# ak110/object_detector

Measured on AMD Instinct MI355X. Metric: images_per_sec, higher is better.
Workload: dtype f16

## Files before the change

### object_detector_amd/csrc/conv_bneck.hip

```cpp
#include <stdlib.h>

#include "conv_common.h"

namespace {

struct BneckKP {
  const f16* x;
  const f16* w1;
  const float* s1;
  const float* b1;
  const f16* w3;
  const float* s3;
  const float* b3;
  f16* out;
  const f16* zero;
  int B, H, W;
  int k1stride, k3stride;
  int act;
  float alpha;
  int tiles_x, tiles_y;
};

template <int CPR>
static __device__ __forceinline__ int bn_swz(int row) {
  return CPR == 16 ? ((row & 7) << 1) : (CPR == 8 ? (row & 7) : 3 * ((row >> 2) & 1));
}

template <int ACT>
static __device__ __forceinline__ float bn_act(float v, float alpha) {
  if (ACT == OD_ACT_LEAKY) return od_leaky(v, alpha);
  if (ACT == OD_ACT_ELU) return v > 0.f ? v : alpha * od_expm1_fast(v);
  return v;
}

static __device__ __forceinline__ __amdgpu_buffer_rsrc_t bn_make_rsrc(const void* base, unsigned bytes) {
  return __builtin_amdgcn_make_buffer_rsrc((void*)base, 0, (int)bytes, 0x00020000);
}
static __device__ __forceinline__ void bn_buffer_dma(__amdgpu_buffer_rsrc_t rs, int voff, int soff, char* lds) {
  __builtin_amdgcn_raw_ptr_buffer_load_lds(rs, (__attribute__((address_space(3))) void*)lds, 16, voff, soff, 0, 0);
}

template <int C>
struct BneckCfg {
  static constexpr int CM = C / 2;
  static constexpr int RBX = 2 * C, RBT = C;
  static constexpr int CPX = RBX / 16, CPT = RBT / 16;
  static constexpr int WW = 18, NWP = WW * WW, NWF = 21;
  static constexpr int XW_BYTES = NWF * 16 * RBX;
  static constexpr int TW_BYTES = NWP * RBT;
  static constexpr int W1_BYTES = CM * RBX;
  static constexpr int W3TAP = C * RBT;
  static constexpr bool RESIDENT = (C == 64);
  static constexpr int NXW = RESIDENT ? 2 : 1;
  static constexpr int OFF_XW = 0, OFF_TW = NXW * XW_BYTES, OFF_W1 = OFF_TW + TW_BYTES;
  static constexpr int OFF_W3 = OFF_W1 + W1_BYTES;
  static constexpr int LDS_BYTES = RESIDENT ? OFF_W3 + 9 * W3TAP : OFF_W3 + W3TAP;
  static constexpr int NSLOT = 7;
  static_assert(RESIDENT || (W3TAP == W1_BYTES && 5 * W3TAP <= XW_BYTES), "ring slots must fit the freed regions");
  static constexpr int NF1 = CM / 16, KS1 = C / 32;
  static constexpr int NF3 = C / 16, KS3 = CM / 32;
  static constexpr int NFW = NF3 / 2;
  static constexpr int TAP_DMAS = C * CPT / 512;
  static __host__ __device__ constexpr int slot_off(int slot) {
    return slot == 0 ? OFF_W3 : (slot == 1 ? OFF_W1 : OFF_XW + (slot - 2) * W3TAP);
  }
};

template <int C, int ACT = OD_ACT_LEAKY>
__global__ __launch_bounds__(C == 64 ? 768 : 512, C == 64 ? 3 : 2) void od_bneck(BneckKP p, int ntiles) {
  using Cf = BneckCfg<C>;
  constexpr bool LOADERS = (C == 64);
  constexpr int CM = Cf::CM, RBX = Cf::RBX, RBT = Cf::RBT, CPX = Cf::CPX, CPT = Cf::CPT, WW = Cf::WW, NWP = Cf::NWP;
  constexpr int NF1 = Cf::NF1, KS1 = Cf::KS1, KS3 = Cf::KS3, NFW = Cf::NFW;
  extern __shared__ __attribute__((aligned(16))) char smem[];

  const int tid = threadIdx.x;
  const int lane = tid & 63;
  const int wave = __builtin_amdgcn_readfirstlane(tid >> 6);
  const int l15 = lane & 15, lq = lane >> 4;
  const int tpi = p.tiles_x * p.tiles_y;

  constexpr int XWT = LOADERS ? 256 : 512;
  constexpr int XWR = (NWP * CPX + XWT - 1) / XWT;
  const int xtid = LOADERS ? tid - 512 : tid, xwave = LOADERS ? wave - 8 : wave;
  int xw_rel[XWR], xw_wyx[XWR];
#pragma unroll
  for (int r = 0; r < XWR; ++r) {
    const int q = r * XWT + xtid;
    const int wp = q / CPX, pc = q - wp * CPX;
    const int wy = wp / WW, wx = wp - wy * WW;
    xw_rel[r] = ((wy - 1) * p.W + (wx - 1)) * C + (pc ^ bn_swz<CPX>(wp)) * 8;
    xw_wyx[r] = (q >= 0 && q < NWP * CPX && xtid >= 0) ? ((wy << 8) | wx) : -1;
  }
  auto issue_xwin = [&](int tile, int buf) {
    const int b = tile / tpi;
    const int trem = tile - b * tpi;
    const int tyi = trem / p.tiles_x, txi = trem - tyi * p.tiles_x;
    const int y0 = tyi * 16, x0 = txi * 16;
    const f16* org = p.x + ((long long)(b * p.H + y0) * p.W + x0) * C;
#pragma unroll
    for (int r = 0; r < XWR; ++r) {
      if (xw_wyx[r] >= 0) {
        const int y = y0 - 1 + (xw_wyx[r] >> 8), x = x0 - 1 + (xw_wyx[r] & 255);
        const bool ok = (unsigned)y < (unsigned)p.H && (unsigned)x < (unsigned)p.W;
        const f16* src = ok ? org + xw_rel[r] : p.zero;
        glds16(src, smem + Cf::OFF_XW + buf * Cf::XW_BYTES + (r * XWT + xwave * 64) * 16);
      }
    }
  };
  constexpr int TAPR = (C * CPT + 511) / 512;
  int tap_voff[TAPR];
#pragma unroll
  for (int r = 0; r < TAPR; ++r) {
    const int q = r * 512 + tid;
    const int n = q / CPT, pc = q - n * CPT;
    tap_voff[r] = q < C * CPT ? (n * p.k3stride + (pc ^ bn_swz<CPT>(n)) * 8) * 2 : (int)0x80000000;
  }
  const __amdgpu_buffer_rsrc_t rs_w3 = bn_make_rsrc(p.w3, 256u * (unsigned)p.k3stride * 2u);
  auto load_tap = [&](int tap, int dst_off) {
#pragma unroll
    for (int r = 0; r < TAPR; ++r) {
      char* dst = smem + dst_off + (r * 512 + wave * 64) * 16;
      if ((r + 1) * 512 <= C * CPT) {
        bn_buffer_dma(rs_w3, tap_voff[r], tap * CM * 2, dst);
      } else if (r * 512 + wave * 64 < C * CPT) {
        bn_buffer_dma(rs_w3, tap_voff[r], tap * CM * 2, dst);
      }
    }
  };

  int tile = blockIdx.x;
  if (tile >= ntiles) return;
  if (LOADERS && wave >= 8) {
    issue_xwin(tile, 0);
    wait_vmcnt<0>();
    __syncthreads();
    int curl = 0;
#pragma unroll 1
    for (; tile < ntiles; tile += (int)gridDim.x) {
      if (tile + (int)gridDim.x < ntiles) issue_xwin(tile + (int)gridDim.x, curl ^ 1);
      __builtin_amdgcn_s_barrier();
      wait_vmcnt<0>();
      __builtin_amdgcn_s_barrier();
      curl ^= 1;
    }
    return;
  }
  if (!LOADERS) issue_xwin(tile, 0);
#pragma unroll 1
  for (int q = tid; q < CM * CPX + 63; q += 512) {
    if (q < CM * CPX) {
      const int n = q / CPX, pc = q - n * CPX;
      const int lc = pc ^ bn_swz<CPX>(n);
      glds16(p.w1 + (long long)n * p.k1stride + lc * 8, smem + Cf::OFF_W1 + (q - lane) * 16);
    }
  }
  if (Cf::RESIDENT) {
#pragma unroll 1
    for (int tap = 0; tap < 9; ++tap) load_tap(tap, Cf::OFF_W3 + tap * Cf::W3TAP);
  } else {
    load_tap(0, Cf::slot_off(0));
  }
  wait_vmcnt<0>();
  __syncthreads();

  const int wm = wave >> 1, wn = wave & 1;
  int boff[NFW][KS3];
#pragma unroll
  for (int j = 0; j < NFW; ++j)
#pragma unroll
    for (int ks = 0; ks < KS3; ++ks) {
      const int row = (wn * NFW + j) * 16 + l15;
      boff[j][ks] = row * RBT + (((ks * 4 + lq) ^ bn_swz<CPT>(row)) * 16);
    }

  int cur = 0;
#pragma unroll 1
  for (; tile < ntiles; tile += (int)gridDim.x) {
    const int b = tile / tpi;
    const int trem = tile - b * tpi;
    const int tyi = trem / p.tiles_x, txi = trem - tyi * p.tiles_x;
    const int y0 = tyi * 16, x0 = txi * 16;
    const char* xw = smem + Cf::OFF_XW + cur * Cf::XW_BYTES;

    {
    f16x8 wb1[NF1][KS1];
  #pragma unroll
    for (int j = 0; j < NF1; ++j)
  #pragma unroll
      for (int ks = 0; ks < KS1; ++ks) {
        const int row = j * 16 + l15;
        wb1[j][ks] = *(const f16x8*)(smem + Cf::OFF_W1 + row * RBX + (((ks * 4 + lq) ^ bn_swz<CPX>(row)) * 16));
      }
    float sc1[NF1][4], bi1[NF1][4];
  #pragma unroll
    for (int j = 0; j < NF1; ++j) {
      const f32x4 s = *(const f32x4*)(p.s1 + j * 16 + lq * 4), bb = *(const f32x4*)(p.b1 + j * 16 + lq * 4);
  #pragma unroll
      for (int e = 0; e < 4; ++e) {
        sc1[j][e] = s[e];
        bi1[j][e] = bb[e];
      }
    }
  #pragma unroll 1
      for (int f = wave; f < Cf::NWF; f += 8) {
        const int wp = f * 16 + l15;
        f32x4 acc1[NF1];
  #pragma unroll
        for (int j = 0; j < NF1; ++j) acc1[j] = f32x4{0.f, 0.f, 0.f, 0.f};
  #pragma unroll
        for (int ks = 0; ks < KS1; ++ks) {
          const f16x8 xa = *(const f16x8*)(xw + wp * RBX + (((ks * 4 + lq) ^ bn_swz<CPX>(wp)) * 16));
  #pragma unroll
          for (int j = 0; j < NF1; ++j) acc1[j] = __builtin_amdgcn_mfma_f32_16x16x32_f16(wb1[j][ks], xa, acc1[j], 0, 0, 0);
        }
        if (wp < NWP) {
          const int wy = wp / WW, wx = wp - wy * WW;
          const bool inside = (unsigned)(y0 - 1 + wy) < (unsigned)p.H && (unsigned)(x0 - 1 + wx) < (unsigned)p.W;
  #pragma unroll
          for (int j = 0; j < NF1; ++j) {
            f16x4 h;
  #pragma unroll
            for (int e = 0; e < 4; ++e) {
              const float v = bn_act<ACT>(acc1[j][e] * sc1[j][e] + bi1[j][e], p.alpha);
              h[e] = inside ? (f16)v : (f16)0.f;
            }
            const int lc = j * 2 + (lq >> 1);
            *(f16x4*)(smem + Cf::OFF_TW + wp * RBT + ((lc ^ bn_swz<CPT>(wp)) * 16) + (lq & 1) * 8) = h;
          }
        }
      }

    }

    f16x8 resv[NFW / 2][4];
    if (!Cf::RESIDENT) {
#pragma unroll
      for (int pr = 0; pr < NFW / 2; ++pr) {
        const int ch = (wn * NFW + 2 * pr + (lq & 1)) * 16 + (lq >> 1) * 8;
#pragma unroll
        for (int i = 0; i < 4; ++i) {
          const int wrow = (wm * 4 + i + 1) * WW + 1 + l15;
          resv[pr][i] = *(const f16x8*)(xw + wrow * RBX + (((ch >> 3) ^ bn_swz<CPX>(wrow)) * 16));
        }
      }
    }
    __syncthreads();

    if (Cf::RESIDENT) {
      if (!LOADERS && tile + (int)gridDim.x < ntiles) issue_xwin(tile + (int)gridDim.x, cur ^ 1);
    } else {
#pragma unroll
      for (int k = 1; k <= 6; ++k) load_tap((k % 3) * 3 + k / 3, Cf::slot_off(k));
    }

    f32x4 acc[4][NFW];
#pragma unroll
    for (int i = 0; i < 4; ++i)
#pragma unroll
      for (int j = 0; j < NFW; ++j) acc[i][j] = f32x4{0.f, 0.f, 0.f, 0.f};

    f16x8 xa[6][KS3];
    auto load_col = [&](int dx) {
#pragma unroll
      for (int k = 0; k < 6; ++k) {
        const int wrow = (wm * 4 + k) * WW + dx + l15;
#pragma unroll
        for (int ks = 0; ks < KS3; ++ks)
          xa[k][ks] = *(const f16x8*)(smem + Cf::OFF_TW + wrow * RBT + (((ks * 4 + lq) ^ bn_swz<CPT>(wrow)) * 16));
      }
    };
    auto do_tap = [&](int dy, int wbase) {
#pragma unroll
      for (int ks = 0; ks < KS3; ++ks) {
        f16x8 wb[NFW];
#pragma unroll
        for (int j = 0; j < NFW; ++j) wb[j] = *(const f16x8*)(smem + wbase + boff[j][ks]);
#pragma unroll
        for (int i = 0; i < 4; ++i)
#pragma unroll
          for (int j = 0; j < NFW; ++j)
            acc[i][j] = __builtin_amdgcn_mfma_f32_16x16x32_f16(wb[j], xa[i + dy][ks], acc[i][j], 0, 0, 0);
      }
    };
    if (Cf::RESIDENT) {
#pragma unroll
      for (int dx = 0; dx < 3; ++dx) {
        load_col(dx);
#pragma unroll
        for (int dy = 0; dy < 3; ++dy) do_tap(dy, Cf::OFF_W3 + (dy * 3 + dx) * Cf::W3TAP);
      }
    } else {
      constexpr int D = Cf::TAP_DMAS;
      load_col(0);
      do_tap(0, Cf::slot_off(0));
      wait_vmcnt<5 * D>();
      __builtin_amdgcn_s_barrier();
      load_tap(1 * 3 + 2, Cf::slot_off(0));
      do_tap(1, Cf::slot_off(1));
      wait_vmcnt<5 * D>();
      __builtin_amdgcn_s_barrier();
      load_tap(2 * 3 + 2, Cf::slot_off(1));
      do_tap(2, Cf::slot_off(2));
      wait_vmcnt<5 * D>();
      __builtin_amdgcn_s_barrier();
      load_col(1);
      do_tap(0, Cf::slot_off(3));
      wait_vmcnt<4 * D>();
      __builtin_amdgcn_s_barrier();
      do_tap(1, Cf::slot_off(4));
      wait_vmcnt<3 * D>();
      __builtin_amdgcn_s_barrier();
      do_tap(2, Cf::slot_off(5));
      wait_vmcnt<2 * D>();
      __builtin_amdgcn_s_barrier();
      load_col(2);
      do_tap(0, Cf::slot_off(6));
      wait_vmcnt<1 * D>();
      __builtin_amdgcn_s_barrier();
      do_tap(1, Cf::slot_off(0));
      wait_vmcnt<0>();
      __builtin_amdgcn_s_barrier();
      do_tap(2, Cf::slot_off(1));
    }

    od_mfma_results_ready();
#pragma unroll
    for (int pr = 0; pr < NFW / 2; ++pr) {
      const int ch = (wn * NFW + 2 * pr + (lq & 1)) * 16 + (lq >> 1) * 8;
      float sc[8], bi[8];
      {
        const f32x4 s0 = *(const f32x4*)(p.s3 + ch), s1 = *(const f32x4*)(p.s3 + ch + 4);
        const f32x4 b0 = *(const f32x4*)(p.b3 + ch), b1 = *(const f32x4*)(p.b3 + ch + 4);
#pragma unroll
        for (int e = 0; e < 4; ++e) {
          sc[e] = s0[e];
          sc[4 + e] = s1[e];
          bi[e] = b0[e];
          bi[4 + e] = b1[e];
        }
      }
#pragma unroll
      for (int i = 0; i < 4; ++i) {
        const int ty = wm * 4 + i;
        f16x8 r;
        if (Cf::RESIDENT) {
          const int wrow = (ty + 1) * WW + 1 + l15;
          r = *(const f16x8*)(xw + wrow * RBX + (((ch >> 3) ^ bn_swz<CPX>(wrow)) * 16));
        } else {
          r = resv[pr][i];
        }
        float v[8];
#pragma unroll
        for (int e = 0; e < 4; ++e) {
          float a = acc[i][2 * pr][e], bq = acc[i][2 * pr + 1][e];
          od_permlane16_swap(a, bq);
          v[e] = a;
          v[4 + e] = bq;
        }
        f16x8 h;
#pragma unroll
        for (int e = 0; e < 8; ++e) h[e] = (f16)(bn_act<ACT>(v[e] * sc[e] + bi[e], p.alpha) + (float)r[e]);
        *(f16x8*)(p.out + ((long long)(b * p.H + y0 + ty) * p.W + x0 + l15) * C + ch) = h;
      }
    }
    if (Cf::RESIDENT) {
      if (!LOADERS) wait_vmcnt<(NFW / 2) * 4>();
      __syncthreads();
      cur ^= 1;
    }
  }
}

}

extern "C" int od_bottleneck_supported(int H, int W, int C) {
  return (C == 64 || C == 128) && H > 0 && W > 0 && (H % 16) == 0 && (W % 16) == 0;
}

int od_bottleneck_prepare(od_ctx* ctx, const od_bneck_desc* d, od_launches* L) {
  OD_REQUIRE(ctx && d, "od_bottleneck_fwd: null ctx/desc");
  OD_REQUIRE(d->x && d->w1 && d->scale1 && d->bias1 && d->w3 && d->scale3 && d->bias3 && d->out,
             "od_bottleneck_fwd: null tensor");
  OD_REQUIRE(od_bottleneck_supported(d->H, d->W, d->C),
             "od_bottleneck_fwd: needs C in {64, 128} and H, W multiples of 16 (got C=%d, %dx%d)", d->C, d->H, d->W);
  OD_REQUIRE(d->B > 0 && (long long)d->B * d->H * d->W * d->C < (1LL << 31), "od_bottleneck_fwd: bad batch / tensor too large");
  OD_REQUIRE(d->act >= OD_ACT_LINEAR && d->act <= OD_ACT_ELU, "od_bottleneck_fwd: bad act");
  OD_REQUIRE(d->act != OD_ACT_LEAKY || (d->alpha >= 0.f && d->alpha <= 1.f), "od_bottleneck_fwd: leaky slope must be in [0, 1]");
  BneckKP p;
  p.x = (const f16*)d->x;
  p.w1 = (const f16*)d->w1;
  p.s1 = d->scale1;
  p.b1 = d->bias1;
  p.w3 = (const f16*)d->w3;
  p.s3 = d->scale3;
  p.b3 = d->bias3;
  p.out = (f16*)d->out;
  p.zero = (const f16*)ctx->zero_page;
  p.B = d->B;
  p.H = d->H;
  p.W = d->W;
  p.k1stride = od_round_up(d->C, 64);
  p.k3stride = od_round_up(9 * (d->C / 2), 64);
  p.act = d->act;
  p.alpha = d->alpha;
  p.tiles_x = d->W / 16;
  p.tiles_y = d->H / 16;
  static_assert(OD_ACT_LINEAR == 0 && OD_ACT_LEAKY == 1 && OD_ACT_ELU == 2, "kernel table order");
#define OD_BN(C, ACT) {(const void*)&od_bneck<C, ACT>, "od_bneck<" #C ", " #ACT ">"}
  static const struct {
    const void* fn;
    const char* name;
  } kernels[2][3] = {{OD_BN(64, 0), OD_BN(64, 1), OD_BN(64, 2)}, {OD_BN(128, 0), OD_BN(128, 1), OD_BN(128, 2)}};
#undef OD_BN
  const auto& k = kernels[d->C == 128][d->act];
  const int lds = d->C == 64 ? BneckCfg<64>::LDS_BYTES : BneckCfg<128>::LDS_BYTES;
  if (int rc = od_ensure_lds(ctx, k.fn, (size_t)lds)) return rc;
  const int ntiles = d->B * p.tiles_x * p.tiles_y;
  const int cus = ctx->num_cu;
  const int grid = d->C == 64 ? (ntiles < cus ? ntiles : cus) : ntiles;
  return od_add_launch(L, {k.name, od_issue_kp_int<BneckKP>, k.fn, dim3((unsigned)grid), dim3(d->C == 64 ? 768 : 512), (size_t)lds},
                       od_kp_int<BneckKP>{p, ntiles});
}

extern "C" int od_bottleneck_fwd(od_ctx* ctx, const od_bneck_desc* d, void* stream) {
  return od_prepare_issue(stream, od_bottleneck_prepare, ctx, d);
}
```

Baseline: 21060.

## Make C=128 bottleneck persistent with next-tile window prefetch into freed ring slots

For the C=128 bottleneck kernel, the grid becomes persistent (capped at CU count). Each CTA now streams the next tile's input window into ring slots freed during the 3x3 tap loop, then reloads tap 0 and the 1x1 weights at the end of the iteration. Scale and bias vectors are cached in LDS instead of being read from global memory every tile. The aim is to hide the input-window and weight load latency behind MFMA work, at the cost of much more intricate vmcnt bookkeeping and tighter LDS usage.

```diff
diff --git a/object_detector_amd/csrc/conv_bneck.hip b/object_detector_amd/csrc/conv_bneck.hip
--- a/object_detector_amd/csrc/conv_bneck.hip
+++ b/object_detector_amd/csrc/conv_bneck.hip
@@ -54,9 +54,13 @@
   static constexpr int NXW = RESIDENT ? 2 : 1;
   static constexpr int OFF_XW = 0, OFF_TW = NXW * XW_BYTES, OFF_W1 = OFF_TW + TW_BYTES;
   static constexpr int OFF_W3 = OFF_W1 + W1_BYTES;
-  static constexpr int LDS_BYTES = RESIDENT ? OFF_W3 + 9 * W3TAP : OFF_W3 + W3TAP;
+  static constexpr int OFF_SB = OFF_W3 + W3TAP;
+  static constexpr int LDS_BYTES = RESIDENT ? OFF_W3 + 9 * W3TAP : OFF_SB + (2 * CM + 2 * C) * 4;
   static constexpr int NSLOT = 7;
   static_assert(RESIDENT || (W3TAP == W1_BYTES && 5 * W3TAP <= XW_BYTES), "ring slots must fit the freed regions");
+  static constexpr int XROUNDS = (NWP * CPX + 511) / 512;
+  static_assert(RESIDENT || (CPX == 16 && W3TAP == 2 * 8192 && (XROUNDS - 1) * 8192 == 5 * W3TAP && LDS_BYTES <= 160 * 1024),
+                "window rounds must map onto ring slots 2-6");
   static constexpr int NF1 = CM / 16, KS1 = C / 32;
   static constexpr int NF3 = C / 16, KS3 = CM / 32;
   static constexpr int NFW = NF3 / 2;
@@ -65,6 +69,22 @@
     return slot == 0 ? OFF_W3 : (slot == 1 ? OFF_W1 : OFF_XW + (slot - 2) * W3TAP);
   }
 };
+
+template <int C, int R0, int R1>
+static __device__ __forceinline__ void bn_issue_xwin_rounds(char* smem, const f16* org, const f16* zero, int H, int W, int y0,
+                                                           int x0, int t4, int cs, int wave) {
+  using Cf = BneckCfg<C>;
+  asm volatile("" : "+v"(t4));
+#pragma unroll
+  for (int r = R0; r < R1; ++r) {
+    const int wp = r * 32 + t4;
+    const int wy = wp / Cf::WW, wx = wp - wy * Cf::WW;
+    const bool ok = wp < Cf::NWP && (unsigned)(y0 - 1 + wy) < (unsigned)H && (unsigned)(x0 - 1 + wx) < (unsigned)W;
+    const f16* src = ok ? org + ((wy - 1) * W + (wx - 1)) * C + cs : zero;
+    const int dw = (r + 1) * 32 <= Cf::NWP ? wave : (wave < 4 ? wave : 1 + (wave & 1));
+    glds16(src, smem + Cf::OFF_XW + (r * 512 + dw * 64) * 16);
+  }
+}
 
 template <int C, int ACT = OD_ACT_LEAKY>
 __global__ __launch_bounds__(C == 64 ? 768 : 512, C == 64 ? 3 : 2) void od_bneck(BneckKP p, int ntiles) {
@@ -146,20 +166,48 @@
     }
     return;
   }
-  if (!LOADERS) issue_xwin(tile, 0);
+  const int xs_t4 = tid >> 4, xs_cs = ((tid & 15) ^ bn_swz<CPX>(xs_t4)) * 8;
+  auto tile_org = [&](int t, int& y0, int& x0) {
+    const int b = t / tpi;
+    const int trem = t - b * tpi;
+    const int tyi = trem / p.tiles_x, txi = trem - tyi * p.tiles_x;
+    y0 = tyi * 16;
+    x0 = txi * 16;
+    return p.x + ((long long)(b * p.H + y0) * p.W + x0) * C;
+  };
+  constexpr int W1_DMAS = CM * CPX / 512;
+  auto load_w1 = [&]() {
+    int t = tid;
+    asm volatile("" : "+v"(t));
+#pragma unroll
+    for (int r = 0; r < W1_DMAS; ++r) {
+      const int q = r * 512 + t;
+      const int n = q / CPX, pc = q - n * CPX;
+      glds16(p.w1 + n * p.k1stride + (pc ^ bn_swz<CPX>(n)) * 8, smem + Cf::OFF_W1 + (r * 512 + wave * 64) * 16);
+    }
+  };
+  if (Cf::RESIDENT) {
+    if (!LOADERS) issue_xwin(tile, 0);
 #pragma unroll 1
-  for (int q = tid; q < CM * CPX + 63; q += 512) {
-    if (q < CM * CPX) {
-      const int n = q / CPX, pc = q - n * CPX;
-      const int lc = pc ^ bn_swz<CPX>(n);
-      glds16(p.w1 + (long long)n * p.k1stride + lc * 8, smem + Cf::OFF_W1 + (q - lane) * 16);
-    }
-  }
-  if (Cf::RESIDENT) {
+    for (int q = tid; q < CM * CPX + 63; q += 512) {
+      if (q < CM * CPX) {
+        const int n = q / CPX, pc = q - n * CPX;
+        const int lc = pc ^ bn_swz<CPX>(n);
+        glds16(p.w1 + (long long)n * p.k1stride + lc * 8, smem + Cf::OFF_W1 + (q - lane) * 16);
+      }
+    }
 #pragma unroll 1
     for (int tap = 0; tap < 9; ++tap) load_tap(tap, Cf::OFF_W3 + tap * Cf::W3TAP);
   } else {
+    static_assert(Cf::RESIDENT || (CM * CPX) % 512 == 0, "w1 rounds must be whole");
+    int y0, x0;
+    const f16* org = tile_org(tile, y0, x0);
+    bn_issue_xwin_rounds<C, 0, Cf::XROUNDS>(smem, org, p.zero, p.H, p.W, y0, x0, xs_t4, xs_cs, wave);
+    load_w1();
     load_tap(0, Cf::slot_off(0));
+    float* sb = (float*)(smem + Cf::OFF_SB);
+    if (tid < 2 * CM) sb[tid] = tid < CM ? p.s1[tid] : p.b1[tid - CM];
+    if (tid < 2 * C) sb[2 * CM + tid] = tid < C ? p.s3[tid] : p.b3[tid - C];
   }
   wait_vmcnt<0>();
   __syncthreads();
@@ -183,19 +231,29 @@
     const int y0 = tyi * 16, x0 = txi * 16;
     const char* xw = smem + Cf::OFF_XW + cur * Cf::XW_BYTES;
 
+    int tl15 = l15, tlq = lq;
+    if (!Cf::RESIDENT) asm volatile("" : "+v"(tl15), "+v"(tlq));
+
     {
     f16x8 wb1[NF1][KS1];
   #pragma unroll
     for (int j = 0; j < NF1; ++j)
   #pragma unroll
       for (int ks = 0; ks < KS1; ++ks) {
-        const int row = j * 16 + l15;
-        wb1[j][ks] = *(const f16x8*)(smem + Cf::OFF_W1 + row * RBX + (((ks * 4 + lq) ^ bn_swz<CPX>(row)) * 16));
+        const int row = j * 16 + tl15;
+        wb1[j][ks] = *(const f16x8*)(smem + Cf::OFF_W1 + row * RBX + (((ks * 4 + tlq) ^ bn_swz<CPX>(row)) * 16));
       }
     float sc1[NF1][4], bi1[NF1][4];
   #pragma unroll
     for (int j = 0; j < NF1; ++j) {
-      const f32x4 s = *(const f32x4*)(p.s1 + j * 16 + lq * 4), bb = *(const f32x4*)(p.b1 + j * 16 + lq * 4);
+      f32x4 s, bb;
+      if (Cf::RESIDENT) {
+        s = *(const f32x4*)(p.s1 + j * 16 + tlq * 4);
+        bb = *(const f32x4*)(p.b1 + j * 16 + tlq * 4);
+      } else {
+        s = *(const f32x4*)(smem + Cf::OFF_SB + (j * 16 + tlq * 4) * 4);
+        bb = *(const f32x4*)(smem + Cf::OFF_SB + (CM + j * 16 + tlq * 4) * 4);
+      }
   #pragma unroll
       for (int e = 0; e < 4; ++e) {
         sc1[j][e] = s[e];
@@ -204,13 +262,13 @@
     }
   #pragma unroll 1
       for (int f = wave; f < Cf::NWF; f += 8) {
-        const int wp = f * 16 + l15;
+        const int wp = f * 16 + tl15;
         f32x4 acc1[NF1];
   #pragma unroll
         for (int j = 0; j < NF1; ++j) acc1[j] = f32x4{0.f, 0.f, 0.f, 0.f};
   #pragma unroll
         for (int ks = 0; ks < KS1; ++ks) {
-          const f16x8 xa = *(const f16x8*)(xw + wp * RBX + (((ks * 4 + lq) ^ bn_swz<CPX>(wp)) * 16));
+          const f16x8 xa = *(const f16x8*)(xw + wp * RBX + (((ks * 4 + tlq) ^ bn_swz<CPX>(wp)) * 16));
   #pragma unroll
           for (int j = 0; j < NF1; ++j) acc1[j] = __builtin_amdgcn_mfma_f32_16x16x32_f16(wb1[j][ks], xa, acc1[j], 0, 0, 0);
         }
@@ -225,8 +283,8 @@
               const float v = bn_act<ACT>(acc1[j][e] * sc1[j][e] + bi1[j][e], p.alpha);
               h[e] = inside ? (f16)v : (f16)0.f;
             }
-            const int lc = j * 2 + (lq >> 1);
-            *(f16x4*)(smem + Cf::OFF_TW + wp * RBT + ((lc ^ bn_swz<CPT>(wp)) * 16) + (lq & 1) * 8) = h;
+            const int lc = j * 2 + (tlq >> 1);
+            *(f16x4*)(smem + Cf::OFF_TW + wp * RBT + ((lc ^ bn_swz<CPT>(wp)) * 16) + (tlq & 1) * 8) = h;
           }
         }
       }
@@ -237,21 +295,31 @@
     if (!Cf::RESIDENT) {
 #pragma unroll
       for (int pr = 0; pr < NFW / 2; ++pr) {
-        const int ch = (wn * NFW + 2 * pr + (lq & 1)) * 16 + (lq >> 1) * 8;
+        const int ch = (wn * NFW + 2 * pr + (tlq & 1)) * 16 + (tlq >> 1) * 8;
 #pragma unroll
         for (int i = 0; i < 4; ++i) {
-          const int wrow = (wm * 4 + i + 1) * WW + 1 + l15;
+          const int wrow = (wm * 4 + i + 1) * WW + 1 + tl15;
           resv[pr][i] = *(const f16x8*)(xw + wrow * RBX + (((ch >> 3) ^ bn_swz<CPX>(wrow)) * 16));
         }
       }
     }
     __syncthreads();
 
+    const int ntile = tile + (int)gridDim.x;
+    int ny0 = 0, nx0 = 0;
+    const f16* norg = p.x;
+    int nH = 0;
+    if (!Cf::RESIDENT && ntile < ntiles) {
+      norg = tile_org(ntile, ny0, nx0);
+      nH = p.H;
+    }
+#define OD_BN_XWIN(R0, R1) bn_issue_xwin_rounds<C, R0, R1>(smem, norg, p.zero, nH, p.W, ny0, nx0, xs_t4, xs_cs, wave)
     if (Cf::RESIDENT) {
       if (!LOADERS && tile + (int)gridDim.x < ntiles) issue_xwin(tile + (int)gridDim.x, cur ^ 1);
     } else {
 #pragma unroll
       for (int k = 1; k <= 6; ++k) load_tap((k % 3) * 3 + k / 3, Cf::slot_off(k));
+      OD_BN_XWIN(Cf::XROUNDS - 1, Cf::XROUNDS);
     }
 
     f32x4 acc[4][NFW];
@@ -262,12 +330,14 @@
 
     f16x8 xa[6][KS3];
     auto load_col = [&](int dx) {
+      int cl15 = l15, clq = lq;
+      if (!Cf::RESIDENT) asm volatile("" : "+v"(cl15), "+v"(clq));
 #pragma unroll
       for (int k = 0; k < 6; ++k) {
-        const int wrow = (wm * 4 + k) * WW + dx + l15;
+        const int wrow = (wm * 4 + k) * WW + dx + cl15;
 #pragma unroll
         for (int ks = 0; ks < KS3; ++ks)
-          xa[k][ks] = *(const f16x8*)(smem + Cf::OFF_TW + wrow * RBT + (((ks * 4 + lq) ^ bn_swz<CPT>(wrow)) * 16));
+          xa[k][ks] = *(const f16x8*)(smem + Cf::OFF_TW + wrow * RBT + (((ks * 4 + clq) ^ bn_swz<CPT>(wrow)) * 16));
       }
     };
     auto do_tap = [&](int dy, int wbase) {
@@ -294,44 +364,62 @@
       constexpr int D = Cf::TAP_DMAS;
       load_col(0);
       do_tap(0, Cf::slot_off(0));
-      wait_vmcnt<5 * D>();
+      wait_vmcnt<5 * D + 1>();
       __builtin_amdgcn_s_barrier();
       load_tap(1 * 3 + 2, Cf::slot_off(0));
       do_tap(1, Cf::slot_off(1));
-      wait_vmcnt<5 * D>();
+      wait_vmcnt<5 * D + 1>();
       __builtin_amdgcn_s_barrier();
       load_tap(2 * 3 + 2, Cf::slot_off(1));
       do_tap(2, Cf::slot_off(2));
-      wait_vmcnt<5 * D>();
-      __builtin_amdgcn_s_barrier();
+      wait_vmcnt<5 * D + 1>();
+      __builtin_amdgcn_s_barrier();
+      OD_BN_XWIN(0, 2);
       load_col(1);
       do_tap(0, Cf::slot_off(3));
-      wait_vmcnt<4 * D>();
-      __builtin_amdgcn_s_barrier();
+      wait_vmcnt<4 * D + 3>();
+      __builtin_amdgcn_s_barrier();
+      OD_BN_XWIN(2, 4);
       do_tap(1, Cf::slot_off(4));
-      wait_vmcnt<3 * D>();
-      __builtin_amdgcn_s_barrier();
+      wait_vmcnt<3 * D + 5>();
+      __builtin_amdgcn_s_barrier();
+      OD_BN_XWIN(4, 6);
       do_tap(2, Cf::slot_off(5));
-      wait_vmcnt<2 * D>();
-      __builtin_amdgcn_s_barrier();
+      wait_vmcnt<2 * D + 7>();
+      __builtin_amdgcn_s_barrier();
+      OD_BN_XWIN(6, 8);
       load_col(2);
       do_tap(0, Cf::slot_off(6));
-      wait_vmcnt<1 * D>();
-      __builtin_amdgcn_s_barrier();
+      wait_vmcnt<1 * D + 8>();
+      __builtin_amdgcn_s_barrier();
+      OD_BN_XWIN(8, 10);
       do_tap(1, Cf::slot_off(0));
-      wait_vmcnt<0>();
-      __builtin_amdgcn_s_barrier();
+      wait_vmcnt<10>();
+      __builtin_amdgcn_s_barrier();
+      load_tap(0, Cf::slot_off(0));
       do_tap(2, Cf::slot_off(1));
-    }
-
+      __builtin_amdgcn_s_barrier();
+      load_w1();
+    }
+#undef OD_BN_XWIN
+
+    int el15 = l15, elq = lq;
+    if (!Cf::RESIDENT) asm volatile("" : "+v"(el15), "+v"(elq));
     od_mfma_results_ready();
 #pragma unroll
     for (int pr = 0; pr < NFW / 2; ++pr) {
-      const int ch = (wn * NFW + 2 * pr + (lq & 1)) * 16 + (lq >> 1) * 8;
+      const int ch = (wn * NFW + 2 * pr + (elq & 1)) * 16 + (elq >> 1) * 8;
       float sc[8], bi[8];
       {
-        const f32x4 s0 = *(const f32x4*)(p.s3 + ch), s1 = *(const f32x4*)(p.s3 + ch + 4);
-        const f32x4 b0 = *(const f32x4*)(p.b3 + ch), b1 = *(const f32x4*)(p.b3 + ch + 4);
+        f32x4 s0, s1, b0, b1;
+        if (Cf::RESIDENT) {
+          s0 = *(const f32x4*)(p.s3 + ch), s1 = *(const f32x4*)(p.s3 + ch + 4);
+          b0 = *(const f32x4*)(p.b3 + ch), b1 = *(const f32x4*)(p.b3 + ch + 4);
+        } else {
+          const char* sb3 = smem + Cf::OFF_SB + 2 * CM * 4;
+          s0 = *(const f32x4*)(sb3 + ch * 4), s1 = *(const f32x4*)(sb3 + (ch + 4) * 4);
+          b0 = *(const f32x4*)(sb3 + (C + ch) * 4), b1 = *(const f32x4*)(sb3 + (C + ch + 4) * 4);
+        }
 #pragma unroll
         for (int e = 0; e < 4; ++e) {
           sc[e] = s0[e];
@@ -345,7 +433,7 @@
         const int ty = wm * 4 + i;
         f16x8 r;
         if (Cf::RESIDENT) {
-          const int wrow = (ty + 1) * WW + 1 + l15;
+          const int wrow = (ty + 1) * WW + 1 + el15;
           r = *(const f16x8*)(xw + wrow * RBX + (((ch >> 3) ^ bn_swz<CPX>(wrow)) * 16));
         } else {
           r = resv[pr][i];
@@ -361,13 +449,16 @@
         f16x8 h;
 #pragma unroll
         for (int e = 0; e < 8; ++e) h[e] = (f16)(bn_act<ACT>(v[e] * sc[e] + bi[e], p.alpha) + (float)r[e]);
-        *(f16x8*)(p.out + ((long long)(b * p.H + y0 + ty) * p.W + x0 + l15) * C + ch) = h;
+        *(f16x8*)(p.out + ((long long)(b * p.H + y0 + ty) * p.W + x0 + el15) * C + ch) = h;
       }
     }
     if (Cf::RESIDENT) {
       if (!LOADERS) wait_vmcnt<(NFW / 2) * 4>();
       __syncthreads();
       cur ^= 1;
+    } else {
+      wait_vmcnt<(NFW / 2) * 4>();
+      __builtin_amdgcn_s_barrier();
     }
   }
 }
@@ -418,7 +509,7 @@
   if (int rc = od_ensure_lds(ctx, k.fn, (size_t)lds)) return rc;
   const int ntiles = d->B * p.tiles_x * p.tiles_y;
   const int cus = ctx->num_cu;
-  const int grid = d->C == 64 ? (ntiles < cus ? ntiles : cus) : ntiles;
+  const int grid = ntiles < cus ? ntiles : cus;
   return od_add_launch(L, {k.name, od_issue_kp_int<BneckKP>, k.fn, dim3((unsigned)grid), dim3(d->C == 64 ? 768 : 512), (size_t)lds},
                        od_kp_int<BneckKP>{p, ntiles});
 }
```

New measurement: 21120, median of 2. No clear change (+0.3%).
